# skokec/DAU-ConvNet

Hardware: AMD Instinct MI355X
Metric: DAU fwd+bwd GSamples/s (N*H*W/s) (higher is better)
Workload: dtype f32

## Files before the change

dau-convnet_amd/csrc/dau_conv_api.hip:

```cpp
#include <cmath>
#include <cstdarg>
#include <cstdio>
#include <algorithm>
#include <atomic>
#include <cstring>
#include <memory>
#include <mutex>
#include <new>
#include <string>
#include <utility>
#include <vector>

#include "dau_common.hpp"
#include "dau_tiled.hpp"

using namespace dau;

namespace {

thread_local std::string g_last_error;

int fail(int code, const char* fmt, ...) {
    char buf[512];
    va_list ap;
// ... 636 lines not shown
    }
    return DAU_OK;
}

int dau_conv_plan_get_info(const dau_conv_plan* plan, dau_conv_plan_info* info) {
    if (!plan || !info) return fail(DAU_INVALID_ARGUMENT, "null argument");
    info->offset_bucket = plan->bucket;
    info->blur_support = plan->blur_k;
    info->algo_forward = plan->algo_fwd;
    info->algo_backward = plan->algo_bwd;
    info->drop_last_col = plan->drop_col;
    info->drop_last_row = plan->drop_row;
    const BucketSet& top = plan->top();
    const bool* s0 = plan->sets[0].has;
    const bool tiled_fwd = plan->algo_fwd == DAU_ALGO_TILED;
    info->gather_patch = tiled_fwd ? top.tiled[kFwd].tiles_x * top.tiled[kFwd].tile_w : 0;
    info->gather_stack = tiled_fwd ? top.tiled[kFwd].stack : 0;
    info->dot_windows = plan->algo_bwd == DAU_ALGO_TILED ? top.tiled_dot.windows : 0;
    info->gather_windows = tiled_fwd ? top.tiled[kFwd].windows : 0;
    info->bucket_sets = plan->dynamic ? plan->nsets : 1;
    const bool dense_reachable = s0[kBf16R4] && (plan->nsets == 1 || plan->dynamic);
    info->gather_dense_bf16 = dense_reachable ? (s0[kWgradR4] ? 2 : 1) : 0;
    info->batch_slab_gather = top.slab_gather;
    info->batch_slab_dot = top.slab_dot;
    info->dot_region = top.has[kTiledDot] ? top.tiled_dot.region_cols * 100 + top.tiled_dot.region_rows : 0;
    info->gather_fblock = tiled_fwd ? top.tiled[kFwd].fblock : 0;
    info->gather_variant = tiled_fwd ? top.tiled[kFwd].variant : -1;
    info->dense_bf16_radius3 = dense_reachable && plan->dynamic && s0[kBf16R3] ? (s0[kWgradR3] ? 2 : 1) : 0;
    info->gather_dense_split = 0;
    if (plan->dynamic && tiled_fwd)
        for (int m = kSplit2; m <= kSplit4; ++m)
            if (s0[m]) info->gather_dense_split |= 1 << kRadius[m];
    if (plan->sets[0].ring) info->gather_dense_split |= 1 << 5;
    if (plan->dynamic && tiled_fwd && s0[kLine4]) info->gather_dense_split |= 1 << 6;
    if (plan->dynamic && tiled_fwd && s0[kLine8]) info->gather_dense_split |= 1 << 7;
    return DAU_OK;
}

int dau_conv_split_dot_geometry(const dau_conv_plan* plan, int32_t* region_width, int32_t* strip_items, int32_t* strip_k_steps) {
    if (!plan) return fail(DAU_INVALID_ARGUMENT, "null argument");
    int rw = 0, items = 0, steps = 0;
    for (int i = 0; i < plan->nsets && !rw; ++i) {
        const BucketSet& bs = plan->sets[i];
        if (!bs.has[kSplitDot]) continue;
        rw = bs.sdot.RW;
        split_dot_strip(bs.sdot, &items, &steps);
    }
    if (region_width) *region_width = rw;
    if (strip_items) *strip_items = items;
    if (strip_k_steps) *strip_k_steps = steps;
    return DAU_OK;
}

int dau_conv_workspace_bytes(const dau_conv_plan* plan, int pass, size_t* bytes_out) {
    if (!plan || !bytes_out) return fail(DAU_INVALID_ARGUMENT, "null argument");
    if (pass == DAU_PASS_FORWARD) *bytes_out = carve_forward(plan, nullptr).bytes;
    else if (pass == DAU_PASS_BACKWARD) *bytes_out = carve_backward(plan, nullptr).bytes;
    else if (pass == DAU_PASS_EPILOGUE_BACKWARD)
        *bytes_out = epilogue_grad_workspace_bytes(plan->sh.N, plan->sh.F, plan->sh.H, plan->sh.W, plan->act(), plan->d.flags & DAU_FLAG_IO_NHWC);
    else return fail(DAU_INVALID_ARGUMENT, "pass must be DAU_PASS_FORWARD, DAU_PASS_BACKWARD or DAU_PASS_EPILOGUE_BACKWARD");
    return DAU_OK;
}

namespace {
int forward_pass(const dau_conv_plan* p, void* stream, const float* x, const float* w, const float* mu1,
                 const float* mu2, const float* sigma, float* y, void* workspace, size_t workspace_bytes, const Epilogue& epi) {
    if (!p || !x || !w || !mu1 || !mu2 || !sigma || !y || !workspace) return fail(DAU_INVALID_ARGUMENT, "null argument");
    FwdWs ws = carve_forward(p, workspace);
    if (workspace_bytes < ws.bytes)
        return fail(DAU_INVALID_ARGUMENT, "workspace too small: %zu < %zu", workspace_bytes, ws.bytes);
    hipStream_t st = static_cast<hipStream_t>(stream);
    if (int rc = ensure_attrs(p)) return rc;
    DAU_HIP(hipMemsetAsync(ws.status, 0, sizeof(Status), st));
    launch_synth_filters(st, sigma, p->blur_k, p->d.flags, ws.filters);
    launch_prepare_units(st, w, mu1, mu2, p->sh, p->d.number_units_ignore, p->d.flags, p->bucket, false, ws.table, ws.status,
                         p->host_status, -1, p->sets[0].has[kLine4] ? ws.status : nullptr);
    run_gather_sum(p, st, kFwd, x, y, ws.filters, ws.table, ws.status, ws.gather, epi);
    DAU_HIP(hipPeekAtLastError());
    return DAU_OK;
}
}

int dau_conv_forward(const dau_conv_plan* p, void* stream, const float* x, const float* w, const float* mu1,
                     const float* mu2, const float* sigma, float* y, void* workspace, size_t workspace_bytes) {
    return forward_pass(p, stream, x, w, mu1, mu2, sigma, y, workspace, workspace_bytes, Epilogue{});
}

int dau_conv_epilogue_supported(const dau_conv_plan* p, int epilogue) {
    if (!p) return fail(DAU_INVALID_ARGUMENT, "null argument");
    if (epilogue & ~(DAU_EPILOGUE_BIAS | DAU_EPILOGUE_RELU))
        return fail(DAU_INVALID_ARGUMENT, "unknown epilogue bits 0x%x (DAU_EPILOGUE_BIAS | DAU_EPILOGUE_RELU)", epilogue);
    if (p->algo_fwd != DAU_ALGO_TILED)
        return fail(DAU_INVALID_ARGUMENT, "the direct kernels take no fused epilogue (this plan's forward pass runs on them)");
    if (p->d.flags & DAU_FLAG_DENSE_BF16)
        return fail(DAU_INVALID_ARGUMENT, "DAU_FLAG_DENSE_BF16 plans take no fused epilogue (the bf16-product forms have none)");
    return DAU_OK;
}

int dau_conv_forward_epilogue(const dau_conv_plan* p, void* stream, const float* x, const float* w, const float* mu1,
                              const float* mu2, const float* sigma, const float* bias, int epilogue, float* y,
                              void* workspace, size_t workspace_bytes) {
    if (epilogue == 0) return forward_pass(p, stream, x, w, mu1, mu2, sigma, y, workspace, workspace_bytes, Epilogue{});
    if (int rc = dau_conv_epilogue_supported(p, epilogue)) return rc;
    if ((epilogue & DAU_EPILOGUE_BIAS) && !bias) return fail(DAU_INVALID_ARGUMENT, "DAU_EPILOGUE_BIAS without a bias");
    Epilogue epi;
    epi.bias = (epilogue & DAU_EPILOGUE_BIAS) ? bias : nullptr;
// ... 228 lines not shown
```

dau-convnet_amd/csrc/dau_tiled.hpp:

```cpp
#pragma once
#include "dau_common.hpp"

namespace dau {

struct TiledConfig {
    int N, Cin, Cout, G, H, W;
    int R;
    int blur_k;
    int NP;
    int windows;
    int stack;
    int patches;
    int rows, pitch;
    int tiles_x, tiles_y;
    int tile_w;
    int fblock;
    int variant;
    int debug;
    int act;
    int nhwc;
    int in_relu;
};

bool tiled_gather_configure(int N, int Cin, int Cout, int G, int H, int W, int R, int blur_k, int act, TiledConfig* cfg);
// ... 55 lines not shown
                          const Epilogue& epi = Epilogue{});
}
struct RingConfig {
    int N, Cin, Cout, G, H, W;
    int nchunk;
    int capacity;
};
void ring_configure(const DenseConfig& dense, long max_outlier_units, RingConfig* cfg);
size_t ring_workspace_bytes(const RingConfig& cfg);
void ring_build_list(hipStream_t st, const RingConfig& cfg, const UnitRef* table, void* workspace, const Guard& guard);
void ring_run(hipStream_t st, const RingConfig& cfg, const SplitStaged& staged, void* workspace, Status* status, const Guard& guard);
float* ring_partial(const RingConfig& cfg, void* workspace);
void ring_init();

struct TiledDotConfig {
    Shape sh;
    int R, blur_k;
    int NP;
    int variant;
    int windows;
    bool as1, one_tile;
    bool rw8;
    bool ring;
    int region_cols, region_rows;
    int rounds;
    int act;
    int ignore;
    int debug;
    int nhwc;
    int in_relu;
};

bool tiled_dot_configure(const Shape& sh, int R, int blur_k, int act, int ignore, TiledDotConfig* cfg);
size_t tiled_dot_workspace_bytes(const TiledDotConfig& cfg);
void tiled_dot_prepare(hipStream_t st, const TiledDotConfig& cfg, const float* x, const float* dy,
                       const float* filters, const UnitRef* table_bare, int drop_col, int drop_row, void* workspace,
                       const Guard& guard);
void tiled_dot_run(hipStream_t st, const TiledDotConfig& cfg, float* r4, void* workspace, const Guard& guard, bool accumulate);
void tiled_dot_init(const TiledDotConfig& cfg);

void launch_blur4_pack(hipStream_t st, const float* x, const float* filters, int N, int C, int cstride, int H, int W, int Hp,
                       int Wp, int blur_k, int act, float* xk, const Guard& guard, unsigned* kmax = nullptr, bool nhwc = false,
                       bool in_relu = false);
void blur4_pack_init(int blur_k, bool kmax = false, bool nhwc = false);
bool blur4_pack_fits(int blur_k, int Hp, int Wp);

void launch_dot_reduce(hipStream_t st, const void* partial, int partial_f32, long n, int G, int F, int g_split, int slabs0,
                       int slabs1, int zero_from, bool accumulate, float* r4, const Guard& guard);

struct SplitDotConfig {
    Shape sh;
    int blur_k;
    int RW;
    int act;
    int e_limbs;
    int nhwc;
    int in_relu;
};
bool split_dot_configure(const Shape& sh, int blur_k, int act, SplitDotConfig* cfg);
size_t split_dot_workspace_bytes(const SplitDotConfig& cfg);
void split_dot_strip(const SplitDotConfig& cfg, int* items, int* k_steps);
void split_dot_init(const SplitDotConfig& cfg);
void split_dot_prepare(hipStream_t st, const SplitDotConfig& cfg, const float* x, const float* dy, const float* filters,
                       int drop_col, int drop_row, void* workspace, const Guard& guard);
void split_dot_run(hipStream_t st, const SplitDotConfig& cfg, const UnitRef* table, float* r4, void* workspace, const Guard& guard);

struct WgradConfig {
    Shape sh;
    int blur_k;
    int SB, FB, NC;
    int HsT, WsT, WT, nseg;
    int splits;
    int Hp, Wp;
    bool fused;
};
#define DAU_DECLARE_DENSE_WGRAD(NS)                                                                                            \
    namespace NS {                                                                                                            \
    bool dense_wgrad_configure(const Shape& sh, int blur_k, bool bf16, WgradConfig* cfg);                                     \
    size_t dense_wgrad_workspace_bytes(const WgradConfig& cfg);                                                               \
    void dense_wgrad_init(const WgradConfig& cfg);                                                                            \
    void dense_wgrad_run(hipStream_t st, const WgradConfig& cfg, const float* x, const float* dy, const float* filters,       \
                         const UnitRef* table, int drop_col, int drop_row, float* r4, void* workspace, const Guard& guard, int nk); \
    }
DAU_DECLARE_DENSE_WGRAD(r4)
DAU_DECLARE_DENSE_WGRAD(r3)

size_t epilogue_grad_workspace_bytes(long N, int F, int H, int W, int act, bool nhwc);
bool epilogue_grad_run(hipStream_t st, long N, int F, int H, int W, int act, bool nhwc, const float* dy, const float* y, bool relu,
                       float* dz, float* dbias, void* workspace);

}
```

dau-convnet_amd/csrc/k_split_dot.hip:

```cpp
#include <algorithm>
#include <cfloat>

#include "dau_tiled.hpp"

namespace dau {

typedef _Float16 h8 __attribute__((ext_vector_type(8)));
typedef float f4s __attribute__((ext_vector_type(4)));

namespace {

constexpr int kSdWaves = 8;
constexpr int kSdAS = 2;
constexpr int kSdGT = 4;
constexpr int kSdSB = kSdWaves * kSdAS;
constexpr int kSdFB = 16;
constexpr int kSdR = 4;
constexpr int kSdRH = 4;
constexpr int kSdFlushItems = 16;
constexpr unsigned kVmcnt0 = 0x0F70, kVmcnt8 = 0x0F78;

inline size_t rup(size_t v, size_t a = 256) { return (v + a - 1) / a * a; }

#ifdef DAU_SD_NO_THIN
constexpr bool kSdThin = false;
#else
constexpr bool kSdThin = true;
#endif

struct SdGeom {
    int Hq, Wq, rq, cq, XTr, XTc, EYs, EXs, octs, nfb, nsb, ngb, items, chunks, per, NP;
    int thin;
    int strip_steps;
};

SdGeom sd_geom(const SplitDotConfig& c) {
    const Shape& s = c.sh;
    SdGeom g{};
    g.Hq = (s.H + 1 + kSdRH - 1) / kSdRH * kSdRH;
    g.Wq = (s.W + 1 + c.RW - 1) / c.RW * c.RW;
    g.rq = g.Hq / kSdRH; g.cq = g.Wq / c.RW;
    g.thin = kSdThin && (s.H + 1) % kSdRH == 1 && g.rq >= 2;
    g.strip_steps = (g.rq - g.thin) * c.RW + g.thin * ((c.RW + kSdRH - 1) / kSdRH);
    g.XTr = g.Hq + 1; g.XTc = g.Wq + 1;
    g.EYs = g.Hq + 2 * kSdR; g.EXs = g.Wq + 2 * kSdR;
    g.octs = (s.N + 7) / 8;
    g.NP = (s.N + 1) / 2;
    g.nfb = (s.F + kSdFB - 1) / kSdFB;
    g.nsb = (s.S + kSdSB - 1) / kSdSB;
    g.ngb = (s.G + kSdGT - 1) / kSdGT;
    g.items = g.octs * g.rq * g.cq;
    const int per_chunk = g.nfb * g.nsb * g.ngb;
    int chunks = (1024 + per_chunk - 1) / per_chunk;
    chunks = std::max(1, std::min(chunks, g.items));
    g.per = (g.items + chunks - 1) / chunks;
    g.chunks = (g.items + g.per - 1) / g.per;
    return g;
}

struct SdLayout { size_t maxes_off, xk_off, xs_off, es_off, partial_off, total; };

SdLayout sd_layout(const SplitDotConfig& c, const SdGeom& g) {
    const Shape& s = c.sh;
    SdLayout l{};
    size_t off = 0;
    l.maxes_off = off; off += rup((size_t)(s.S * kNumK + s.F) * 4);
    l.xk_off = off; off += rup((size_t)g.NP * s.S * s.H * s.W * 32);
    l.xs_off = off; off += rup((size_t)g.octs * s.S * kNumK * g.XTr * g.XTc * 32 + 32);
    l.es_off = off; off += rup((size_t)g.octs * g.nfb * g.EYs * g.EXs * 256 * c.e_limbs);
    l.partial_off = off; off += rup((size_t)g.chunks * kNumK * s.S * s.G * s.F * 4);
    l.total = off;
    return l;
}

__device__ __forceinline__ int sd_shift(unsigned maxbits) {
    if (maxbits == 0u) return 0;
    const int e = (int)(maxbits >> 23) - 127;
    const int sh = 13 - e;
    return sh > 120 ? 120 : sh;
}

__device__ __forceinline__ bool finite_abs(float v, float* a) {
    *a = fabsf(v);
    return *a <= FLT_MAX;
}

#ifdef DAU_SD_STAGE_REF
__global__ void __launch_bounds__(256) sd_absmax_x_kernel(const float* __restrict__ xk, int NP, int S, int HW, int split,
                                                          unsigned* __restrict__ xmax, const Guard guard) {
    if (!guard_pass(guard)) return;
    const int s = blockIdx.x % S, part = blockIdx.x / S;
    float m[4] = {0.0f, 0.0f, 0.0f, 0.0f};
    const long per_np = (long)HW * 2;
    const long total = (long)NP * per_np;
    for (long i = part * 256L + threadIdx.x; i < total; i += 256L * split) {
        const long np = i / per_np, r = i - np * per_np;
        const float4 v = reinterpret_cast<const float4*>(xk + ((size_t)np * S + s) * HW * 8)[r];
        const int k0 = (int)(r & 1) * 2;
        float a;
        if (finite_abs(v.x, &a)) m[k0] = fmaxf(m[k0], a);
        if (finite_abs(v.y, &a)) m[k0] = fmaxf(m[k0], a);
        if (finite_abs(v.z, &a)) m[k0 + 1] = fmaxf(m[k0 + 1], a);
        if (finite_abs(v.w, &a)) m[k0 + 1] = fmaxf(m[k0 + 1], a);
    }
    __shared__ float red[4][256];
    for (int k = 0; k < 4; ++k) red[k][threadIdx.x] = m[k];
    __syncthreads();
    for (int w = 128; w >= 1; w >>= 1) {
        if ((int)threadIdx.x < w)
// ... 869 lines not shown
void launch_sd(hipStream_t st, const SdArgs* a, int grid) {
    auto kern = [] { if constexpr (EL == 2) return split_gather_dot_kernel<RW>; else return sd_e1_dot_kernel<RW>; }();
    const size_t lds = (size_t)(2 * kSdRH + 2 * kSdR) * (RW + 2 * kSdR) * 256 * EL;
    if (!a) { (void)hipFuncSetAttribute(reinterpret_cast<const void*>(kern), hipFuncAttributeMaxDynamicSharedMemorySize, 160 * 1024); return; }
    hipLaunchKernelGGL(kern, dim3(grid), dim3(kSdWaves * 64), lds, st, *a);
}
bool sd_walks(const SplitDotConfig& c) {
#if defined(DAU_SD_XK_COPY) || defined(DAU_SD_STAGE_REF)
    return false;
#else
    const SdGeom g = sd_geom(c);
    const long nct = (g.XTc + kXwCols - 1) / kXwCols;
    return !c.nhwc && (c.blur_k == 5 || c.blur_k == 7 || c.blur_k == 9) && (long)g.octs * c.sh.S * nct < (1L << 31);
#endif
}
template <int K, bool STORE>
void launch_xk_walk(hipStream_t st, const XkWalkArgs& a, int grid) {
    hipLaunchKernelGGL((sd_xk_walk_kernel<K, STORE>), dim3(grid), dim3(64), 0, st, a);
}
template <bool STORE>
void dispatch_xk_walk(hipStream_t st, const SplitDotConfig& c, const SdGeom& g, const float* x, const float* filters, unsigned* xmax,
                      h8* xs, const Guard& guard) {
    XkWalkArgs a{};
    a.x = x; a.taps = filters + kTaps1dOffset; a.xmax = xmax; a.xs = xs;
    a.N = c.sh.N; a.S = c.sh.S; a.H = c.sh.H; a.W = c.sh.W; a.XTr = g.XTr; a.XTc = g.XTc; a.act = c.act; a.relu_in = c.in_relu;
    a.nct = (g.XTc + kXwCols - 1) / kXwCols;
    a.guard = guard;
    const int grid = g.octs * c.sh.S * a.nct;
    if (c.blur_k == 5) launch_xk_walk<5, STORE>(st, a, grid);
    else if (c.blur_k == 7) launch_xk_walk<7, STORE>(st, a, grid);
    else launch_xk_walk<9, STORE>(st, a, grid);
}

void dispatch_sd(int RW, int e_limbs, hipStream_t st, const SdArgs* a, int grid) {
    if (e_limbs == 1) {
        if (RW == 10) launch_sd<10, 1>(st, a, grid);
        else launch_sd<12, 1>(st, a, grid);
    } else {
        if (RW == 10) launch_sd<10, 2>(st, a, grid);
        else launch_sd<12, 2>(st, a, grid);
    }
}

}

bool split_dot_configure(const Shape& sh, int blur_k, int act, SplitDotConfig* cfg) {
    int best = 0;
    long best_cost = 1L << 40;
    for (int rw = 12; rw >= 10; rw -= 2) {
        const long wq = (sh.W + 1 + rw - 1) / rw * rw;
        const long cost = wq * (rw + 2) * (60 / rw);
        if (cost < best_cost) { best_cost = cost; best = rw; }
    }
    if ((size_t)(2 * kSdRH + 2 * kSdR) * (best + 2 * kSdR) * 512 > 160 * 1024) return false;
    if (!blur4_pack_fits(blur_k, sh.H, sh.W)) return false;
    SplitDotConfig c{};
    c.sh = sh; c.blur_k = blur_k; c.RW = best; c.act = act;
#ifdef DAU_SD_BF16_E2
    c.e_limbs = 2;
#else
    c.e_limbs = act == kActBF16 ? 1 : 2;
#endif
    const SdGeom g = sd_geom(c);
    if ((long)g.EXs * 512 * 32 > (1L << 31)) return false;
    *cfg = c;
    return true;
}

size_t split_dot_workspace_bytes(const SplitDotConfig& c) { return sd_layout(c, sd_geom(c)).total; }

void split_dot_strip(const SplitDotConfig& c, int* items, int* k_steps) {
    const SdGeom g = sd_geom(c);
    *items = g.rq; *k_steps = g.strip_steps;
}

void split_dot_init(const SplitDotConfig& c) {
    dispatch_sd(c.RW, c.e_limbs, nullptr, nullptr, 0);
#ifndef DAU_SD_STAGE_REF
    blur4_pack_init(c.blur_k, true, c.nhwc != 0);
#else
    blur4_pack_init(c.blur_k, false, c.nhwc != 0);
#endif
}

void split_dot_prepare(hipStream_t st, const SplitDotConfig& c, const float* x, const float* dy, const float* filters,
                       int drop_col, int drop_row, void* workspace, const Guard& guard) {
    const SdGeom g = sd_geom(c);
    const SdLayout l = sd_layout(c, g);
    const Shape& s = c.sh;
    char* ws = static_cast<char*>(workspace);
    unsigned* xmax = reinterpret_cast<unsigned*>(ws + l.maxes_off);
    unsigned* emax = xmax + s.S * kNumK;
    float* xk = reinterpret_cast<float*>(ws + l.xk_off);
    (void)hipMemsetAsync(xmax, 0, (size_t)(s.S * kNumK + s.F) * 4, st);
    (void)hipMemsetAsync(ws + l.partial_off, 0, (size_t)g.chunks * kNumK * s.S * s.G * s.F * 4, st);
    const int HW = s.H * s.W;
    const bool walks = sd_walks(c);
    h8* xs = reinterpret_cast<h8*>(ws + l.xs_off);
#ifndef DAU_SD_STAGE_REF
    if (walks) dispatch_xk_walk<false>(st, c, g, x, filters, xmax, xs, guard);
    else launch_blur4_pack(st, x, filters, s.N, s.S, s.S, s.H, s.W, s.H, s.W, c.blur_k, c.act, xk, guard, xmax, c.nhwc != 0, c.in_relu != 0);
#else
    launch_blur4_pack(st, x, filters, s.N, s.S, s.S, s.H, s.W, s.H, s.W, c.blur_k, c.act, xk, guard, nullptr, c.nhwc != 0, c.in_relu != 0);
    const int xsplit = std::max(1, std::min(16, 2048 / std::max(1, s.S)));
    hipLaunchKernelGGL(sd_absmax_x_kernel, dim3(s.S * xsplit), dim3(256), 0, st, xk, g.NP, s.S, HW, xsplit, xmax, guard);
#endif
    if (c.nhwc) {
        const int nfb64 = (s.F + 63) / 64;
        const int esplit = (int)std::max(1L, std::min((long)(2048 / nfb64), ((long)s.N * HW + 3) / 4));
        hipLaunchKernelGGL(sd_absmax_nhwc_e_kernel, dim3(nfb64 * esplit), dim3(256), 0, st, dy, s.N, s.F, HW, esplit, c.act, emax, guard);
    } else {
        const int esplit = std::max(1, std::min(16, 2048 / std::max(1, s.F)));
        hipLaunchKernelGGL(sd_absmax_e_kernel, dim3(s.F * esplit), dim3(256), 0, st, dy, s.N, s.F, HW, esplit, c.act, emax, guard);
    }
    if (walks) dispatch_xk_walk<true>(st, c, g, x, filters, xmax, xs, guard);
    else hipLaunchKernelGGL(sd_stage_x_kernel, dim3(8192), dim3(256), 0, st, xk, xmax, s.N, g.NP, s.S, s.H, s.W, g.octs, g.XTr, g.XTc, xs, guard);
    if (c.e_limbs == 1) {
        const int nct = (g.EXs + kSe1TX - 1) / kSe1TX, tx = (g.EXs + nct - 1) / nct;
        if (c.nhwc) {
            hipLaunchKernelGGL(sd_stage_nhwc_e_kernel<1>, dim3((unsigned)(g.octs * g.nfb * g.EYs * nct)), dim3(256), 0, st, dy, emax, s.N, s.F,
                               s.H, s.W, g.nfb, g.EYs, g.EXs, nct, tx, drop_col, drop_row, c.act, reinterpret_cast<h8*>(ws + l.es_off), guard);
            return;
        }
        hipLaunchKernelGGL(sd_stage_e1_kernel, dim3((unsigned)(g.octs * g.nfb * g.EYs * nct)), dim3(256), 0, st, dy, emax, s.N, s.F,
                           s.H, s.W, g.nfb, g.EYs, g.EXs, nct, tx, drop_col, drop_row, c.act, reinterpret_cast<h8*>(ws + l.es_off), guard);
        return;
    }
#ifndef DAU_SD_STAGE_REF
    const int nct = (g.EXs + kSeTX - 1) / kSeTX, tx = (g.EXs + nct - 1) / nct;
    if (c.nhwc) {
        hipLaunchKernelGGL(sd_stage_nhwc_e_kernel<2>, dim3((unsigned)(g.octs * g.nfb * g.EYs * nct)), dim3(256), 0, st, dy, emax, s.N, s.F,
                           s.H, s.W, g.nfb, g.EYs, g.EXs, nct, tx, drop_col, drop_row, c.act, reinterpret_cast<h8*>(ws + l.es_off), guard);
        return;
    }
#ifndef DAU_SD_STAGE_E_ROWS
    SeWalkArgs w{};
    w.dy = dy; w.emax = emax; w.es = reinterpret_cast<h8*>(ws + l.es_off);
    w.N = s.N; w.F = s.F; w.H = s.H; w.W = s.W; w.nfb = g.nfb; w.EYs = g.EYs; w.EXs = g.EXs;
    w.nct = (g.EXs + kSeCols - 1) / kSeCols;
    w.wlim = drop_col ? s.W - 1 : s.W; w.hlim = drop_row ? s.H - 1 : s.H; w.act = c.act; w.guard = guard;
    const long cols = (long)g.octs * g.nfb * w.nct, nb = (5120 + cols - 1) / cols;
    const int rb = DAU_TUNE_INT("DAU_SD_STAGE_E_RB", 0);
    w.RB = rb > 0 ? rb : std::max(4, (int)((g.EYs + nb - 1) / nb));
    w.nbands = (g.EYs + w.RB - 1) / w.RB;
    hipLaunchKernelGGL(sd_stage_e_kernel, dim3((unsigned)(cols * w.nbands)), dim3(64), 0, st, w);
    return;
#else
    hipLaunchKernelGGL(sd_stage_e_kernel, dim3((unsigned)(g.octs * g.nfb * g.EYs * nct)), dim3(256), 0, st, dy, emax, s.N, s.F, s.H,
                       s.W, g.nfb, g.EYs, g.EXs, nct, tx, drop_col, drop_row, c.act, reinterpret_cast<h8*>(ws + l.es_off), guard);
#endif
#else
    hipLaunchKernelGGL(sd_stage_e_kernel, dim3(4096), dim3(256), 0, st, dy, emax, s.N, s.F, s.H, s.W, g.octs, g.nfb, g.EYs, g.EXs,
                       drop_col, drop_row, c.act, c.nhwc, reinterpret_cast<h8*>(ws + l.es_off), guard);
#endif
}

void split_dot_run(hipStream_t st, const SplitDotConfig& c, const UnitRef* table, float* r4, void* workspace, const Guard& guard) {
    const SdGeom g = sd_geom(c);
    const SdLayout l = sd_layout(c, g);
    const Shape& s = c.sh;
    char* ws = static_cast<char*>(workspace);
    SdArgs a{};
    a.xs = reinterpret_cast<const h8*>(ws + l.xs_off);
    a.es = ws + l.es_off;
    a.xmax = reinterpret_cast<const unsigned*>(ws + l.maxes_off);
    a.emax = a.xmax + s.S * kNumK;
    a.table = table;
    a.partial = reinterpret_cast<float*>(ws + l.partial_off);
    a.S = s.S; a.F = s.F; a.G = s.G;
    a.nfb = g.nfb; a.nsb = g.nsb; a.ngb = g.ngb; a.per = g.per; a.items = g.items; a.rq = g.rq; a.cq = g.cq;
    a.XTr = g.XTr; a.XTc = g.XTc; a.EYs = g.EYs; a.EXs = g.EXs;
    a.thin = g.thin;
    a.guard = guard;
    dispatch_sd(c.RW, c.e_limbs, st, &a, g.chunks * g.nfb * g.nsb * g.ngb);
    launch_dot_reduce(st, a.partial, 1, (long)kNumK * s.S * s.G * s.F, s.G, s.F, s.G, g.chunks, g.chunks, s.G, false, r4, guard);
}

}
```

dau-convnet_amd/dau_conv/_capi.py:

```python
import ctypes
import os

import torch

_HERE = os.path.dirname(os.path.abspath(__file__))
_LIB_PATH = os.environ.get("DAU_CONV_LIB") or os.path.join(_HERE, "libdau_conv_hip.so")

DAU_OK, DAU_INVALID_ARGUMENT, DAU_FAILED_PRECONDITION, DAU_INTERNAL = 0, 1, 2, 3

FLAG_USE_INTERPOLATION = 1 << 0
FLAG_UNIT_TESTING = 1 << 1
FLAG_SINGLE_DIM_KERNEL = 1 << 2
FLAG_FORBID_POSITIVE_DIM1 = 1 << 3
FLAG_IO_BF16 = 1 << 4
FLAG_STATIC_BUCKET = 1 << 5
FLAG_DENSE_BF16 = 1 << 6
FLAG_DENSE_WGRAD_NEVER = 1 << 7
FLAG_DENSE_WGRAD_ALWAYS = 1 << 8
FLAG_DENSE_SPLIT_F16 = 1 << 9
FLAG_NO_DENSE_SPLIT = 1 << 10
FLAG_DENSE_SPLIT_LINE = 1 << 15
FLAG_DENSE_SPLIT_OUTLIERS = 1 << 12
FLAG_IO_F16 = 1 << 11
FLAG_IO_NHWC = 1 << 13
# ... 12 lines not shown
class InvalidArgumentError(DAUConvError, ValueError):
    code = DAU_INVALID_ARGUMENT


class FailedPreconditionError(DAUConvError):
    code = DAU_FAILED_PRECONDITION


class InternalError(DAUConvError):
    code = DAU_INTERNAL


class _Desc(ctypes.Structure):
    _fields_ = [
        ("struct_size", ctypes.c_int32), ("batch", ctypes.c_int32), ("in_channels", ctypes.c_int32),
        ("out_channels", ctypes.c_int32), ("units_per_channel", ctypes.c_int32), ("height", ctypes.c_int32),
        ("width", ctypes.c_int32), ("max_kernel_size", ctypes.c_int32), ("number_units_ignore", ctypes.c_int32),
        ("flags", ctypes.c_int32), ("algo", ctypes.c_int32), ("sigma_hint", ctypes.c_float),
        ("mu_learning_rate_factor", ctypes.c_float),
    ]


class _Info(ctypes.Structure):
    _fields_ = [(n, ctypes.c_int32) for n in
                ("offset_bucket", "blur_support", "algo_forward", "algo_backward", "drop_last_col", "drop_last_row",
                 "gather_patch", "gather_stack", "dot_windows", "gather_windows", "bucket_sets", "gather_dense_bf16", "batch_slab_gather", "batch_slab_dot", "dot_region", "gather_fblock", "gather_variant", "dense_bf16_radius3", "gather_dense_split")]


def _load():
    if not os.path.exists(_LIB_PATH):
        raise ImportError(
            "dau_conv: %s not found. Build it with `make -C dau-convnet_amd/csrc` (hipcc, gfx950) or "
            "`python -c 'import __graft_entry__ as g; g.build()'`. There is no CPU fallback." % _LIB_PATH)
    lib = ctypes.CDLL(_LIB_PATH)
    vp, fp, ip = ctypes.c_void_p, ctypes.c_void_p, ctypes.c_void_p
    lib.dau_conv_abi_version.restype = ctypes.c_int
    lib.dau_conv_last_error.restype = ctypes.c_char_p
    lib.dau_conv_build_id.restype = ctypes.c_char_p
    lib.dau_conv_plan_create.argtypes = [ctypes.POINTER(_Desc), ctypes.POINTER(vp)]
    lib.dau_conv_plan_destroy.argtypes = [vp]
    lib.dau_conv_plan_get_info.argtypes = [vp, ctypes.POINTER(_Info)]
    lib.dau_conv_workspace_bytes.argtypes = [vp, ctypes.c_int, ctypes.POINTER(ctypes.c_size_t)]
    lib.dau_conv_forward.argtypes = [vp, vp, fp, fp, fp, fp, fp, fp, vp, ctypes.c_size_t]
    lib.dau_conv_backward.argtypes = [vp, vp] + [fp] * 11 + [vp, ctypes.c_size_t, ctypes.c_int]
    lib.dau_conv_backward_param_sums.argtypes = [vp, vp] + [fp] * 6 + [vp, ctypes.c_size_t]
    lib.dau_conv_finalize_param_grads.argtypes = [vp, vp] + [fp] * 6 + [ctypes.c_int]
    lib.dau_conv_check_status.argtypes = [vp, vp, vp, ctypes.POINTER(ctypes.c_float)]
    if hasattr(lib, "dau_conv_gather_outlier_status"):
        lib.dau_conv_gather_outlier_status.argtypes = [vp, vp, vp, ctypes.POINTER(ctypes.c_int32), ctypes.POINTER(ctypes.c_int32)]
    if hasattr(lib, "dau_conv_gather_line_status"):
        lib.dau_conv_gather_line_status.argtypes = [vp, vp, vp, ctypes.POINTER(ctypes.c_int32), ctypes.POINTER(ctypes.c_int32)]
    if hasattr(lib, "dau_conv_split_dot_geometry"):
        lib.dau_conv_split_dot_geometry.argtypes = [vp] + [ctypes.POINTER(ctypes.c_int32)] * 3
    if hasattr(lib, "dau_conv_forward_epilogue"):
        lib.dau_conv_epilogue_supported.argtypes = [vp, ctypes.c_int]
        lib.dau_conv_forward_epilogue.argtypes = [vp, vp, fp, fp, fp, fp, fp, fp, ctypes.c_int, fp, vp, ctypes.c_size_t]
        lib.dau_conv_epilogue_backward.argtypes = [vp, vp, fp, fp, ctypes.c_int, fp, fp, vp, ctypes.c_size_t]
    if hasattr(lib, "dau_conv_forward_residual"):
        lib.dau_conv_forward_residual.argtypes = [vp, vp, fp, fp, fp, fp, fp, fp, fp, ctypes.c_int, fp, vp, ctypes.c_size_t]
    lib.dau_conv_last_status.argtypes = [vp, ctypes.POINTER(ctypes.c_float), ctypes.POINTER(ctypes.c_int32)]
    lib.dau_conv_filters.argtypes = [vp, vp, fp, fp]
    lib.dau_conv_unit_table.argtypes = [vp, vp, fp, fp, fp, ctypes.c_int, vp]
    lib.dau_conv_filter_support.argtypes = [ctypes.c_float]
    lib.dau_conv_filter_support.restype = ctypes.c_int
    lib.dau_conv_profile_begin.argtypes = [vp]
    lib.dau_conv_profile_end.argtypes = [vp, ctypes.POINTER(ctypes.c_double), ctypes.POINTER(ctypes.c_int32)]
    if lib.dau_conv_abi_version() != 4:
        raise ImportError("dau_conv: ABI version mismatch in %s" % _LIB_PATH)
    return lib


lib = _load()


def filter_support(sigma):
    return int(lib.dau_conv_filter_support(ctypes.c_float(float(sigma))))


def build_id():
    return lib.dau_conv_build_id().decode()


def _check(code):
    if code == DAU_OK:
        return
    msg = lib.dau_conv_last_error().decode("utf-8", "replace")
    raise {DAU_INVALID_ARGUMENT: InvalidArgumentError, DAU_FAILED_PRECONDITION: FailedPreconditionError}.get(
        code, InternalError)(msg)


def _ptr(t):
    return None if t is None else ctypes.c_void_p(t.data_ptr())


def _stream(device):
    return ctypes.c_void_p(torch.cuda.current_stream(device).cuda_stream)


def _same_device(*tensors):
    dev = tensors[0].device
    for t in tensors[1:]:
        if t is not None and t.device != dev:
            raise InvalidArgumentError("all tensors of a call must be on the same device (%s vs %s)" % (dev, t.device))
    return dev


# ... 149 lines not shown
        return dx, dw, dmu1, dmu2, dsigma

    def backward_param_sums(self, x, dy, mu1, mu2, sigma, out=None):
        pshape = (1, self.S, self.G, self.F)
        _req(x, "input", (self.N, self.S, self.H, self.W), self.io_dtype, self._io_format)
        _req(dy, "grad", (self.N, self.F, self.H, self.W), self.io_dtype, self._io_format)
        for t, n in ((mu1, "mu1"), (mu2, "mu2"), (sigma, "sigma")):
            _req(t, n, pshape)
        dev = _same_device(x, dy, mu1, mu2, sigma, out)
        with torch.cuda.device(dev):
            if out is None:
                out = torch.empty((4, self.S, self.G, self.F), dtype=torch.float32, device=dev)
            _req(out, "sums", (4, self.S, self.G, self.F))
            ws = self._workspace(PASS_BACKWARD, dev)
            _check(lib.dau_conv_backward_param_sums(self._h, _stream(dev), _ptr(x), _ptr(dy), _ptr(mu1), _ptr(mu2), _ptr(sigma),
                                                    _ptr(out), _ptr(ws), ws.numel()))
        self._last_ws = ws
        return out

    def finalize_param_grads(self, sums, w, need_mask=NEED_DW | NEED_DMU1 | NEED_DMU2 | NEED_DSIGMA):
        pshape = (1, self.S, self.G, self.F)
        _req(sums, "sums", (4, self.S, self.G, self.F))
        _req(w, "weights", pshape)
        dev = _same_device(sums, w)
        new = lambda: torch.empty(pshape, dtype=torch.float32, device=dev)
        with torch.cuda.device(dev):
            dw = new() if need_mask & NEED_DW else None
            dmu1 = new() if need_mask & NEED_DMU1 else None
            dmu2 = new() if need_mask & NEED_DMU2 else None
            dsigma = new() if need_mask & NEED_DSIGMA else None
            _check(lib.dau_conv_finalize_param_grads(self._h, _stream(dev), _ptr(sums), _ptr(w), _ptr(dw), _ptr(dmu1),
                                                     _ptr(dmu2), _ptr(dsigma), int(need_mask)))
        return dw, dmu1, dmu2, dsigma

    def check_status(self):
        mx = ctypes.c_float()
        dev = self._last_ws.device
        with torch.cuda.device(dev):
            _check(lib.dau_conv_check_status(self._h, _stream(dev), _ptr(self._last_ws), ctypes.byref(mx)))
        return mx.value

    def outlier_status(self):
        units, taken = ctypes.c_int32(), ctypes.c_int32()
        dev = self._last_ws.device
        with torch.cuda.device(dev):
            _check(lib.dau_conv_gather_outlier_status(self._h, _stream(dev), _ptr(self._last_ws), ctypes.byref(units), ctypes.byref(taken)))
        return units.value, bool(taken.value)

    def split_dot_geometry(self):
        v = [ctypes.c_int32() for _ in range(3)]
        _check(lib.dau_conv_split_dot_geometry(self._h, *[ctypes.byref(c) for c in v]))
        return tuple(c.value for c in v)

    def line_status(self):
        units, taken = ctypes.c_int32(), ctypes.c_int32()
        dev = self._last_ws.device
        with torch.cuda.device(dev):
            _check(lib.dau_conv_gather_line_status(self._h, _stream(dev), _ptr(self._last_ws), ctypes.byref(units), ctypes.byref(taken)))
        return units.value, taken.value

    def last_status(self):
        mx, valid = ctypes.c_float(), ctypes.c_int32()
        _check(lib.dau_conv_last_status(self._h, ctypes.byref(mx), ctypes.byref(valid)))
        return mx.value if valid.value else None

    def profile_begin(self):
        _check(lib.dau_conv_profile_begin(self._h))

    def profile_end(self):
        ms = (ctypes.c_double * 3)()
        n = (ctypes.c_int32 * 3)()
        _check(lib.dau_conv_profile_end(self._h, ms, n))
        return {name: (ms[i], n[i]) for i, name in enumerate(("gather_sum_fwd", "gather_sum_dx", "gather_dot"))}

    def filters(self, sigma):
        k = self.info["blur_support"]
        out = torch.empty((6, k, k), dtype=torch.float32, device=sigma.device)
        with torch.cuda.device(sigma.device):
            _check(lib.dau_conv_filters(self._h, _stream(sigma.device), _ptr(sigma), _ptr(out)))
        return out

    def unit_table(self, mu1, mu2, w=None, form=0):
        units = self.S * self.G * self.F
        raw = torch.empty((units, 6), dtype=torch.int32, device=mu1.device)
        with torch.cuda.device(mu1.device):
            _check(lib.dau_conv_unit_table(self._h, _stream(mu1.device), _ptr(w), _ptr(mu1), _ptr(mu2), int(form), _ptr(raw)))
        return raw[:, :2].contiguous(), raw[:, 2:].contiguous().view(torch.float32)
```

include/dau_conv.h:

```cpp
#ifndef DAU_CONV_H_
#define DAU_CONV_H_

#include <stddef.h>
#include <stdint.h>

#ifdef __cplusplus
extern "C" {
#endif

#define DAU_CONV_ABI_VERSION 4

#if defined(__GNUC__)
#define DAU_API __attribute__((visibility("default")))
#else
#define DAU_API
#endif

enum {
    DAU_OK = 0,
    DAU_INVALID_ARGUMENT = 1,
    DAU_FAILED_PRECONDITION = 2,
    DAU_INTERNAL = 3
};

// ... 39 lines not shown
    DAU_NEED_ALL = 31
};

typedef struct dau_conv_desc {
    int32_t struct_size;
    int32_t batch;
    int32_t in_channels;
    int32_t out_channels;
    int32_t units_per_channel;
    int32_t height, width;
    int32_t max_kernel_size;
    int32_t number_units_ignore;
    int32_t flags;
    int32_t algo;
    float sigma_hint;
    float mu_learning_rate_factor;
} dau_conv_desc;

typedef struct dau_conv_plan dau_conv_plan;

typedef struct dau_conv_plan_info {
    int32_t offset_bucket;
    int32_t blur_support;
    int32_t algo_forward;
    int32_t algo_backward;
    int32_t drop_last_col;
    int32_t drop_last_row;
    int32_t gather_patch;
    int32_t gather_stack;
    int32_t dot_windows;
    int32_t gather_windows;
    int32_t bucket_sets;
    int32_t gather_dense_bf16;
    int32_t batch_slab_gather;
    int32_t batch_slab_dot;
    int32_t dot_region;
    int32_t gather_fblock;
    int32_t gather_variant;
    int32_t dense_bf16_radius3;
    int32_t gather_dense_split;
} dau_conv_plan_info;

DAU_API int dau_conv_abi_version(void);
DAU_API const char *dau_conv_build_id(void);
DAU_API const char *dau_conv_last_error(void);

DAU_API int dau_conv_filter_support(float sigma);

DAU_API int dau_conv_plan_create(const dau_conv_desc *desc, dau_conv_plan **plan_out);
DAU_API int dau_conv_plan_destroy(dau_conv_plan *plan);
DAU_API int dau_conv_plan_get_info(const dau_conv_plan *plan, dau_conv_plan_info *info);
DAU_API int dau_conv_workspace_bytes(const dau_conv_plan *plan, int pass, size_t *bytes_out);
DAU_API int dau_conv_split_dot_geometry(const dau_conv_plan *plan, int32_t *region_width, int32_t *strip_items, int32_t *strip_k_steps);

DAU_API int dau_conv_forward(const dau_conv_plan *plan, void *stream, const float *x, const float *w,
                     const float *mu1, const float *mu2, const float *sigma, float *y,
                     void *workspace, size_t workspace_bytes);

DAU_API int dau_conv_epilogue_supported(const dau_conv_plan *plan, int epilogue);
DAU_API int dau_conv_forward_epilogue(const dau_conv_plan *plan, void *stream, const float *x, const float *w,
                     const float *mu1, const float *mu2, const float *sigma, const float *bias, int epilogue,
                     float *y, void *workspace, size_t workspace_bytes);

DAU_API int dau_conv_forward_residual(const dau_conv_plan *plan, void *stream, const float *x, const float *w,
                     const float *mu1, const float *mu2, const float *sigma, const float *bias, const float *residual,
                     int epilogue, float *y, void *workspace, size_t workspace_bytes);

DAU_API int dau_conv_epilogue_backward(const dau_conv_plan *plan, void *stream, const float *dy, const float *y, int epilogue,
                     float *dz, float *dbias, void *workspace, size_t workspace_bytes);

DAU_API int dau_conv_backward(const dau_conv_plan *plan, void *stream, const float *x, const float *dy,
                      const float *w, const float *mu1, const float *mu2, const float *sigma,
                      float *dx, float *dw, float *dmu1, float *dmu2, float *dsigma,
                      void *workspace, size_t workspace_bytes, int need_mask);

DAU_API int dau_conv_backward_param_sums(const dau_conv_plan *plan, void *stream, const float *x, const float *dy,
                                 const float *mu1, const float *mu2, const float *sigma, float *sums_out,
                                 void *workspace, size_t workspace_bytes);
DAU_API int dau_conv_finalize_param_grads(const dau_conv_plan *plan, void *stream, const float *sums, const float *w,
                                  float *dw, float *dmu1, float *dmu2, float *dsigma, int need_mask);

DAU_API int dau_conv_check_status(const dau_conv_plan *plan, void *stream, const void *workspace,
                          float *max_abs_mu_out);

DAU_API int dau_conv_gather_outlier_status(const dau_conv_plan *plan, void *stream, const void *workspace,
                                   int32_t *outlier_units, int32_t *ring_taken);

DAU_API int dau_conv_gather_line_status(const dau_conv_plan *plan, void *stream, const void *workspace,
                                int32_t *off_line_units, int32_t *line_radius_taken);

DAU_API int dau_conv_last_status(const dau_conv_plan *plan, float *max_abs_mu_out, int32_t *valid_out);

DAU_API int dau_conv_filters(const dau_conv_plan *plan, void *stream, const float *sigma, float *filters_out);
DAU_API int dau_conv_unit_table(const dau_conv_plan *plan, void *stream, const float *w, const float *mu1, const float *mu2,
                        int form, void *table_out);

enum { DAU_PROFILE_SLOTS = 3 };
DAU_API int dau_conv_profile_begin(dau_conv_plan *plan);
DAU_API int dau_conv_profile_end(dau_conv_plan *plan, double *ms_out, int32_t *passes_out);

#ifdef __cplusplus
}
#endif
#endif
```

Baseline: 0.01862.

## Cover split-dot columns with mixed 12- and 10-wide region groups

The split-dot backward kernel now tiles the padded width with a mix of 12-wide and 10-wide column regions, chosen to minimise padded columns plus halo overhead, instead of a single region width. Each group is launched as its own kernel instance with its own chunking, and the result goes into a shared partial buffer that is reduced afterwards. This cuts wasted padded work when the width is not a multiple of the best region width. The cost is up to two launches per pass, a possible imbalance between the two groups' chunk counts, and a workspace fit check that now assumes the wider region.

```diff
diff --git a/dau-convnet_amd/csrc/dau_conv_api.hip b/dau-convnet_amd/csrc/dau_conv_api.hip
--- a/dau-convnet_amd/csrc/dau_conv_api.hip
+++ b/dau-convnet_amd/csrc/dau_conv_api.hip
@@ -712,6 +712,23 @@
     return DAU_OK;
 }
 
+int dau_conv_split_dot_cover(const dau_conv_plan* plan, int32_t widths[2], int32_t strips[2], int32_t strip_k_steps[2]) {
+    if (!plan) return fail(DAU_INVALID_ARGUMENT, "null argument");
+    int w[2] = {0, 0}, n[2] = {0, 0}, k[2] = {0, 0};
+    for (int i = 0; i < plan->nsets; ++i) {
+        const BucketSet& bs = plan->sets[i];
+        if (!bs.has[kSplitDot]) continue;
+        split_dot_cover(bs.sdot, w, n, k);
+        break;
+    }
+    for (int i = 0; i < 2; ++i) {
+        if (widths) widths[i] = w[i];
+        if (strips) strips[i] = n[i];
+        if (strip_k_steps) strip_k_steps[i] = k[i];
+    }
+    return DAU_OK;
+}
+
 int dau_conv_workspace_bytes(const dau_conv_plan* plan, int pass, size_t* bytes_out) {
     if (!plan || !bytes_out) return fail(DAU_INVALID_ARGUMENT, "null argument");
     if (pass == DAU_PASS_FORWARD) *bytes_out = carve_forward(plan, nullptr).bytes;
diff --git a/dau-convnet_amd/csrc/dau_tiled.hpp b/dau-convnet_amd/csrc/dau_tiled.hpp
--- a/dau-convnet_amd/csrc/dau_tiled.hpp
+++ b/dau-convnet_amd/csrc/dau_tiled.hpp
@@ -131,6 +131,7 @@
     Shape sh;
     int blur_k;
     int RW;
+    int gw[2], gn[2];
     int act;
     int e_limbs;
     int nhwc;
@@ -139,6 +140,7 @@
 bool split_dot_configure(const Shape& sh, int blur_k, int act, SplitDotConfig* cfg);
 size_t split_dot_workspace_bytes(const SplitDotConfig& cfg);
 void split_dot_strip(const SplitDotConfig& cfg, int* items, int* k_steps);
+void split_dot_cover(const SplitDotConfig& cfg, int widths[2], int strips[2], int k_steps[2]);
 void split_dot_init(const SplitDotConfig& cfg);
 void split_dot_prepare(hipStream_t st, const SplitDotConfig& cfg, const float* x, const float* dy, const float* filters,
                        int drop_col, int drop_row, void* workspace, const Guard& guard);
diff --git a/dau-convnet_amd/csrc/k_split_dot.hip b/dau-convnet_amd/csrc/k_split_dot.hip
--- a/dau-convnet_amd/csrc/k_split_dot.hip
+++ b/dau-convnet_amd/csrc/k_split_dot.hip
@@ -7,6 +7,10 @@
 
 typedef _Float16 h8 __attribute__((ext_vector_type(8)));
 typedef float f4s __attribute__((ext_vector_type(4)));
+
+#ifdef DAU_SD_UNIFORM_STRIPS
+__global__ void sd_uniform_strips_build_kernel() {}
+#endif
 
 namespace {
 
@@ -28,10 +32,22 @@
 constexpr bool kSdThin = true;
 #endif
 
+#ifdef DAU_SD_UNIFORM_STRIPS
+constexpr bool kSdCover = false;
+#else
+constexpr bool kSdCover = true;
+#endif
+
+struct SdGroup {
+    int col0, RW, cq;
+    int items, per, chunks;
+    int strip_steps;
+};
+
 struct SdGeom {
-    int Hq, Wq, rq, cq, XTr, XTc, EYs, EXs, octs, nfb, nsb, ngb, items, chunks, per, NP;
+    int Hq, Wq, rq, XTr, XTc, EYs, EXs, octs, nfb, nsb, ngb, chunks, NP;
     int thin;
-    int strip_steps;
+    SdGroup grp[2];
 };
 
 SdGeom sd_geom(const SplitDotConfig& c) {
@@ -39,9 +55,8 @@
     SdGeom g{};
     g.Hq = (s.H + 1 + kSdRH - 1) / kSdRH * kSdRH;
     g.Wq = (s.W + 1 + c.RW - 1) / c.RW * c.RW;
-    g.rq = g.Hq / kSdRH; g.cq = g.Wq / c.RW;
+    g.rq = g.Hq / kSdRH;
     g.thin = kSdThin && (s.H + 1) % kSdRH == 1 && g.rq >= 2;
-    g.strip_steps = (g.rq - g.thin) * c.RW + g.thin * ((c.RW + kSdRH - 1) / kSdRH);
     g.XTr = g.Hq + 1; g.XTc = g.Wq + 1;
     g.EYs = g.Hq + 2 * kSdR; g.EXs = g.Wq + 2 * kSdR;
     g.octs = (s.N + 7) / 8;
@@ -49,12 +64,26 @@
     g.nfb = (s.F + kSdFB - 1) / kSdFB;
     g.nsb = (s.S + kSdSB - 1) / kSdSB;
     g.ngb = (s.G + kSdGT - 1) / kSdGT;
-    g.items = g.octs * g.rq * g.cq;
     const int per_chunk = g.nfb * g.nsb * g.ngb;
-    int chunks = (1024 + per_chunk - 1) / per_chunk;
-    chunks = std::max(1, std::min(chunks, g.items));
-    g.per = (g.items + chunks - 1) / chunks;
-    g.chunks = (g.items + g.per - 1) / g.per;
+    auto chunking = [&](int items, int cap, int* per, int* chunks) {
+        int n = std::max(1, std::min(std::min((1024 + per_chunk - 1) / per_chunk, cap), items));
+        *per = (items + n - 1) / n;
+        *chunks = (items + *per - 1) / *per;
+    };
+    int uni_per, uni_chunks;
+    chunking(g.octs * g.rq * (g.Wq / c.RW), 1 << 30, &uni_per, &uni_chunks);
+    int col = 0;
+    for (int i = 0; i < 2; ++i) {
+        SdGroup& q = g.grp[i];
+        q.col0 = col; q.RW = c.gw[i]; q.cq = c.gn[i];
+        col += q.RW * q.cq;
+        if (!q.cq) continue;
+        q.items = g.octs * g.rq * q.cq;
+        q.strip_steps = (g.rq - g.thin) * q.RW + g.thin * ((q.RW + kSdRH - 1) / kSdRH);
+        chunking(q.items, c.gn[1] ? uni_chunks : 1 << 30, &q.per, &q.chunks);
+        if (i == 1 && DAU_TUNE_INT("DAU_DOT_G2_MATCH", 0)) chunking(q.items, (q.items + g.grp[0].per - 1) / g.grp[0].per, &q.per, &q.chunks);
+        g.chunks = std::max(g.chunks, q.chunks);
+    }
     return g;
 }
 
@@ -1030,10 +1059,30 @@
         const long cost = wq * (rw + 2) * (60 / rw);
         if (cost < best_cost) { best_cost = cost; best = rw; }
     }
-    if ((size_t)(2 * kSdRH + 2 * kSdR) * (best + 2 * kSdR) * 512 > 160 * 1024) return false;
+    const int pin = DAU_TUNE_INT("DAU_DOT_RW", 0);
+    if (pin == 10 || pin == 12) best = pin;
+    if ((size_t)(2 * kSdRH + 2 * kSdR) * (12 + 2 * kSdR) * 512 > 160 * 1024) return false;
     if (!blur4_pack_fits(blur_k, sh.H, sh.W)) return false;
     SplitDotConfig c{};
     c.sh = sh; c.blur_k = blur_k; c.RW = best; c.act = act;
+    const int wq = (sh.W + 1 + best - 1) / best * best;
+    int n[2] = {best == 12 ? wq / 12 : 0, best == 10 ? wq / 10 : 0};
+    if (kSdCover && pin != 10 && pin != 12) {
+        auto has_best = [&](int n12, int n10) { return (best == 12 ? n12 : n10) > 0; };
+        long cover_cost = wq + 2 * (n[0] + n[1]);
+        for (int n12 = 0; 12 * n12 < sh.W + 1 + 12; ++n12) {
+            const int n10 = std::max(0, (sh.W + 1 - 12 * n12 + 9) / 10), cols = 12 * n12 + 10 * n10;
+            if (cols > wq) continue;
+            const long cost = cols + 2 * (n12 + n10);
+            const bool better = cost < cover_cost ||
+                                (cost == cover_cost && (has_best(n12, n10) > has_best(n[0], n[1]) ||
+                                                        (has_best(n12, n10) == has_best(n[0], n[1]) && n12 + n10 < n[0] + n[1])));
+            if (better) { cover_cost = cost; n[0] = n12; n[1] = n10; }
+        }
+    }
+    c.gw[0] = best; c.gn[0] = n[best == 12 ? 0 : 1];
+    c.gw[1] = 22 - best; c.gn[1] = n[best == 12 ? 1 : 0];
+    if (!c.gn[0]) { c.gw[0] = c.gw[1]; c.gn[0] = c.gn[1]; c.gn[1] = 0; }
 #ifdef DAU_SD_BF16_E2
     c.e_limbs = 2;
 #else
@@ -1049,11 +1098,20 @@
 
 void split_dot_strip(const SplitDotConfig& c, int* items, int* k_steps) {
     const SdGeom g = sd_geom(c);
-    *items = g.rq; *k_steps = g.strip_steps;
+    *items = g.rq; *k_steps = g.grp[0].strip_steps;
+}
+
+void split_dot_cover(const SplitDotConfig& c, int widths[2], int strips[2], int k_steps[2]) {
+    const SdGeom g = sd_geom(c);
+    for (int i = 0; i < 2; ++i) {
+        const bool on = g.grp[i].cq > 0;
+        widths[i] = on ? g.grp[i].RW : 0; strips[i] = g.grp[i].cq; k_steps[i] = on ? g.grp[i].strip_steps : 0;
+    }
 }
 
 void split_dot_init(const SplitDotConfig& c) {
-    dispatch_sd(c.RW, c.e_limbs, nullptr, nullptr, 0);
+    for (int i = 0; i < 2; ++i)
+        if (c.gn[i]) dispatch_sd(c.gw[i], c.e_limbs, nullptr, nullptr, 0);
 #ifndef DAU_SD_STAGE_REF
     blur4_pack_init(c.blur_k, true, c.nhwc != 0);
 #else
@@ -1146,11 +1204,20 @@
     a.table = table;
     a.partial = reinterpret_cast<float*>(ws + l.partial_off);
     a.S = s.S; a.F = s.F; a.G = s.G;
-    a.nfb = g.nfb; a.nsb = g.nsb; a.ngb = g.ngb; a.per = g.per; a.items = g.items; a.rq = g.rq; a.cq = g.cq;
+    a.nfb = g.nfb; a.nsb = g.nsb; a.ngb = g.ngb; a.rq = g.rq;
     a.XTr = g.XTr; a.XTc = g.XTc; a.EYs = g.EYs; a.EXs = g.EXs;
     a.thin = g.thin;
     a.guard = guard;
-    dispatch_sd(c.RW, c.e_limbs, st, &a, g.chunks * g.nfb * g.nsb * g.ngb);
+    const h8* xs = a.xs;
+    const char* es = a.es;
+    const int first = g.grp[1].cq && g.grp[1].RW > g.grp[0].RW ? 1 : 0;
+    for (int i = 0; i < 2; ++i) {
+        const SdGroup& q = g.grp[i ^ first];
+        if (!q.cq) continue;
+        a.xs = xs + (size_t)q.col0 * 2; a.es = es + (size_t)q.col0 * 256 * c.e_limbs;
+        a.per = q.per; a.items = q.items; a.cq = q.cq;
+        dispatch_sd(q.RW, c.e_limbs, st, &a, q.chunks * g.nfb * g.nsb * g.ngb);
+    }
     launch_dot_reduce(st, a.partial, 1, (long)kNumK * s.S * s.G * s.F, s.G, s.F, s.G, g.chunks, g.chunks, s.G, false, r4, guard);
 }
 
diff --git a/dau-convnet_amd/dau_conv/_capi.py b/dau-convnet_amd/dau_conv/_capi.py
--- a/dau-convnet_amd/dau_conv/_capi.py
+++ b/dau-convnet_amd/dau_conv/_capi.py
@@ -88,6 +88,8 @@
         lib.dau_conv_gather_line_status.argtypes = [vp, vp, vp, ctypes.POINTER(ctypes.c_int32), ctypes.POINTER(ctypes.c_int32)]
     if hasattr(lib, "dau_conv_split_dot_geometry"):
         lib.dau_conv_split_dot_geometry.argtypes = [vp] + [ctypes.POINTER(ctypes.c_int32)] * 3
+    if hasattr(lib, "dau_conv_split_dot_cover"):
+        lib.dau_conv_split_dot_cover.argtypes = [vp] + [ctypes.POINTER(ctypes.c_int32)] * 3
     if hasattr(lib, "dau_conv_forward_epilogue"):
         lib.dau_conv_epilogue_supported.argtypes = [vp, ctypes.c_int]
         lib.dau_conv_forward_epilogue.argtypes = [vp, vp, fp, fp, fp, fp, fp, fp, ctypes.c_int, fp, vp, ctypes.c_size_t]
@@ -343,6 +345,11 @@
         _check(lib.dau_conv_split_dot_geometry(self._h, *[ctypes.byref(c) for c in v]))
         return tuple(c.value for c in v)
 
+    def split_dot_cover(self):
+        v = [(ctypes.c_int32 * 2)() for _ in range(3)]
+        _check(lib.dau_conv_split_dot_cover(self._h, *v))
+        return tuple(tuple(int(c) for c in a) for a in v)
+
     def line_status(self):
         units, taken = ctypes.c_int32(), ctypes.c_int32()
         dev = self._last_ws.device
diff --git a/include/dau_conv.h b/include/dau_conv.h
--- a/include/dau_conv.h
+++ b/include/dau_conv.h
@@ -115,6 +115,7 @@
 DAU_API int dau_conv_plan_get_info(const dau_conv_plan *plan, dau_conv_plan_info *info);
 DAU_API int dau_conv_workspace_bytes(const dau_conv_plan *plan, int pass, size_t *bytes_out);
 DAU_API int dau_conv_split_dot_geometry(const dau_conv_plan *plan, int32_t *region_width, int32_t *strip_items, int32_t *strip_k_steps);
+DAU_API int dau_conv_split_dot_cover(const dau_conv_plan *plan, int32_t widths[2], int32_t strips[2], int32_t strip_k_steps[2]);
 
 DAU_API int dau_conv_forward(const dau_conv_plan *plan, void *stream, const float *x, const float *w,
                      const float *mu1, const float *mu2, const float *sigma, float *y,
```

After: 0.01879, median of 6. Within noise of the previous version (+0.9%).
